# jwwangchn/BONAI

Measured on AMD Instinct MI355X. Metric: training img/s at 1024x1024 LOFT R50-FPN, higher is better.
Workload: dtype bf16; 1 GPU; LOFT R50-FPN + FOA, 8x1024x1024 synthetic tiles per GPU (BASELINE configs[1]), 80 gt/img, full train step (fwd+losses+bwd+allreduce+clip+SGD), random-init weights, RoI heads at the load of a trained RPN (first proposals = jittered gt boxes); global_batch=8, per_gpu_batch=8, parallelism=dp1, graph_features=False

## Files before the change

### bonai_amd/csrc/elementwise.hip

```cpp
#include "loft_common.h"
#include "../../include/loft_hip.h"
#include "conv_tap.h"

__device__ __forceinline__ void ld8(const bf16_t* p, float v[8]) {
    uint4 t = *reinterpret_cast<const uint4*>(p);
    unpack8_16(t, v);
}
__device__ __forceinline__ void st8(bf16_t* p, const float v[8]) {
    *reinterpret_cast<uint4*>(p) = pack8_16(v);
}

__device__ __forceinline__ void ld8(const float* p, float v[8]) { ld4(p, v); ld4(p + 4, v + 4); }
__device__ __forceinline__ void st8(float* p, const float v[8]) { st4(p, v); st4(p + 4, v + 4); }

static inline dim3 ew_grid(long nvec) {
    long b = (nvec + 255) / 256;
    if (b > 8192) b = 8192;
    if (b < 1) b = 1;
    return dim3((unsigned)b);
}

__global__ void relu_bwd_kernel(const bf16_t* __restrict__ g, const bf16_t* __restrict__ y, bf16_t* __restrict__ out,
                                long nvec) {
    for (long i = blockIdx.x * (long)blockDim.x + threadIdx.x; i < nvec; i += (long)gridDim.x * blockDim.x) {
// ... 625 lines not shown
        const int mid = (lo + hi) >> 1;
        if (e0 < t.end[mid]) hi = mid; else lo = mid + 1;
    }
    while (lo < t.S - 1 && e >= t.end[lo]) ++lo;
    return lo;
}

template <bool NEST, bool TAIL>
__device__ __forceinline__ void sgd_elem(float& pv, float& mv, const float gv, const float s, const float lr, const float mu,
                                         const float wd) {
#pragma clang fp contract(off)
    float d, upd;
    if (TAIL) {
        d = __builtin_fmaf(gv, s, wd * pv);
        mv = mu * mv + d;
        upd = NEST ? d + mu * mv : mv;
    } else {
        d = __builtin_fmaf(wd, pv, gv * s);
        mv = __builtin_fmaf(mu, mv, d);
        upd = NEST ? __builtin_fmaf(mu, mv, d) : mv;
    }
    pv = __builtin_fmaf(-lr, upd, pv);
}
template <bool SEG, bool NEST>
__device__ __forceinline__ void sgd_update(float* __restrict__ p, const float* __restrict__ g, float* __restrict__ m, long n,
                                           float gnorm_sq, float max_norm, float lr, float mu, float wd, float gscale,
                                           const SegTable tab, const long stride, const long t0) {
    float clip = 1.f;
    if (max_norm > 0.f) {
        const float norm = sqrtf(gnorm_sq) * gscale;
        if (norm > max_norm) clip = max_norm / (norm + 1e-6f);
    }
    const float s = clip * gscale;
    const bool al = ((reinterpret_cast<uintptr_t>(p) | reinterpret_cast<uintptr_t>(g) | reinterpret_cast<uintptr_t>(m)) & 15) == 0;
    const long n4 = al ? n >> 2 : 0;
    float4* p4 = reinterpret_cast<float4*>(p);
    float4* m4 = reinterpret_cast<float4*>(m);
    const float4* g4 = reinterpret_cast<const float4*>(g);
    const long lane = threadIdx.x & 63;
    auto rates = [&](long e, long first, float& lr_e, float& wd_e) {
        lr_e = lr; wd_e = wd;
        if (SEG) {
            const int sg = seg_find(tab, e, first);
            lr_e = lr * tab.lr_mult[sg]; wd_e = wd * tab.wd_mult[sg];
        }
    };
    auto upd = [&](float4& pv, float4& mv, const float4 gv, long i) {
        float lr_e, wd_e;
        rates(4 * i, 4 * (i - lane), lr_e, wd_e);
        sgd_elem<NEST, false>(pv.x, mv.x, gv.x, s, lr_e, mu, wd_e);
        sgd_elem<NEST, false>(pv.y, mv.y, gv.y, s, lr_e, mu, wd_e);
        sgd_elem<NEST, false>(pv.z, mv.z, gv.z, s, lr_e, mu, wd_e);
        sgd_elem<NEST, false>(pv.w, mv.w, gv.w, s, lr_e, mu, wd_e);
    };
    long i = t0;
    for (; i + stride < n4; i += 2 * stride) {
// ... 265 lines not shown
    if (bias_out && blockIdx.x == 0)
        for (int n = threadIdx.x; n < CoutP; n += blockDim.x) {
            if (n >= Cout) bias_out[n] = 0.f;
            else if (gamma) bias_out[n] = beta[n] - mean[n] * gamma[n] * rsqrtf(var[n] + eps);
            else bias_out[n] = cbias ? cbias[n] : 0.f;
        }
}
LOFT_EXPORT int loft_fold_pack(const float* w, const float* conv_bias, const float* gamma, const float* beta, const float* mean,
                               const float* var, float eps, int Cout, int Cin, int RS, void* wp_fwd, void* wp_dgrad,
                               float* bias_out, int pack_f32, int CoutP, int CinP, void* stream) {
    if (CoutP < Cout || CinP < Cin) return (int)hipErrorInvalidValue;
    const long total = (long)CoutP * CinP * RS;
    if (total <= 0) return 0;
    if (pack_f32)
        hipLaunchKernelGGL(fold_pack_kernel<float>, ew_grid(total), dim3(256), 0, (hipStream_t)stream, w, conv_bias, gamma, beta,
                           mean, var, eps, Cout, Cin, RS, (float*)wp_fwd, (float*)wp_dgrad, bias_out, CoutP, CinP);
    else
        hipLaunchKernelGGL(fold_pack_kernel<bf16_t>, ew_grid(total), dim3(256), 0, (hipStream_t)stream, w, conv_bias, gamma, beta,
                           mean, var, eps, Cout, Cin, RS, (bf16_t*)wp_fwd, (bf16_t*)wp_dgrad, bias_out, CoutP, CinP);
    LOFT_LAUNCH_CHECK();
    return 0;
}

__device__ __forceinline__ int find_record(const long* __restrict__ desc, int n, long key) {
    int cnt = 0;
    for (int j = threadIdx.x & 63; j < n; j += 64) cnt += desc[(long)j * 16 + 15] <= key ? 1 : 0;
    for (int o = 32; o > 0; o >>= 1) cnt += __shfl_xor(cnt, o, 64);
    return cnt - 1;
}

constexpr int FOLD_CHUNK = 2048;
constexpr int FOLD_TILE_MAX_RS = 9;
constexpr int FOLD_NT_TAPS = 32, FOLD_NT_TAPS_LOG2 = 5;
constexpr int FOLD_TILE_FLOATS = FOLD_NT_TAPS * (64 * FOLD_TILE_MAX_RS + 4) / 2;
__global__ __launch_bounds__(256) void fold_pack_multi_kernel(const long* __restrict__ desc, int n, long nchunks) {
    __shared__ float tile[FOLD_TILE_FLOATS];
    for (long c = blockIdx.x; c < nchunks; c += gridDim.x) {
        const int lo = find_record(desc, n, c);
        const long* d = desc + (long)lo * 16;
        const float* w = reinterpret_cast<const float*>(d[0]);
        const float* cbias = reinterpret_cast<const float*>(d[1]);
        const float* gamma = reinterpret_cast<const float*>(d[2]);
        const float* beta = reinterpret_cast<const float*>(d[3]);
        const float* mean = reinterpret_cast<const float*>(d[4]);
        const float* var = reinterpret_cast<const float*>(d[5]);
        bf16_t* wp = reinterpret_cast<bf16_t*>(d[6]);
        bf16_t* wpt = reinterpret_cast<bf16_t*>(d[7]);
        float* bias_out = reinterpret_cast<float*>(d[8]);
        const float eps = __int_as_float((int)d[9]);
        const int Cout = (int)d[10], Cin = (int)d[11], CoutP = (int)d[13], CinP = (int)d[14];
        const bool nmajor = d[12] < 0;
        const int RS = (int)(nmajor ? -d[12] : d[12]);
        const int local_chunk = (int)(c - d[15]);
        if (local_chunk == 0 && bias_out)
            for (int nn = threadIdx.x; nn < CoutP; nn += blockDim.x) {
                if (nn >= Cout) bias_out[nn] = 0.f;
                else if (gamma) bias_out[nn] = beta[nn] - mean[nn] * gamma[nn] * rsqrtf(var[nn] + eps);
                else bias_out[nn] = cbias ? cbias[nn] : 0.f;
            }
        if (nmajor) {
            bf16_t* row = reinterpret_cast<bf16_t*>(tile);
            const int nn = local_chunk, per = Cin * RS;
            const float sc = gamma ? gamma[nn] * rsqrtf(var[nn] + eps) : 1.f;
            __syncthreads();
            const unsigned rs_mul = RS == 1 ? 0u : 0xFFFFFFFFu / (unsigned)RS + 1u;
            const bool small = per < 65536;
            for (int j = threadIdx.x; j < per; j += 256) {
                const int cc = RS == 1 ? j : (small ? (int)__umulhi((unsigned)j, rs_mul) : j / RS), t = j - cc * RS;
                row[t * Cin + cc] = f32_to_bf16(w[(long)nn * per + j] * sc);
            }
            __syncthreads();
            if (wp)
                for (int j = threadIdx.x * 2; j < per; j += 512)
                    *reinterpret_cast<uint32_t*>(wp + (long)nn * per + j) = *reinterpret_cast<const uint32_t*>(row + j);
            continue;
        }
        if (RS > FOLD_TILE_MAX_RS) {
            const long total = (long)CoutP * CinP * RS;
            const long i0 = (long)local_chunk * FOLD_CHUNK;
            for (long i = i0 + threadIdx.x; i < i0 + FOLD_CHUNK && i < total; i += blockDim.x) {
                const int cc = (int)(i % CinP);
                const long r = i / CinP;
                const int nn = (int)(r % CoutP), t = (int)(r / CoutP);
                float v = 0.f;
                if (nn < Cout && cc < Cin) {
                    v = w[((long)nn * Cin + cc) * RS + t];
                    if (gamma) v *= gamma[nn] * rsqrtf(var[nn] + eps);
                }
                const bf16_t h = f32_to_bf16(v);
                if (wp) wp[i] = h;
                if (wpt) wpt[((long)t * CinP + cc) * CoutP + nn] = h;
            }
            continue;
        }
        bf16_t* bt = reinterpret_cast<bf16_t*>(tile);
        const int NT = RS == 1 ? 64 : FOLD_NT_TAPS;
        const int tc = (CinP + 63) >> 6;
        const int n0 = (local_chunk / tc) * NT, c0 = (local_chunk % tc) * 64;
        const int span = 64 * RS, ldw = span + 4;
        __syncthreads();
        const bool vec = (Cin & 63) == 0 && (CinP & 7) == 0 && (CoutP & 7) == 0 && (reinterpret_cast<uintptr_t>(w) & 15) == 0;
        const unsigned rs_mul = RS == 1 ? 0u : 0xFFFFFFFFu / (unsigned)RS + 1u;
        if (vec) {
            const int q4 = span >> 2;
            const unsigned q_mul = 0xFFFFFFFFu / (unsigned)q4 + 1u;
            for (int i = threadIdx.x; i < NT * q4; i += 256) {
                const int row = (int)__umulhi((unsigned)i, q_mul), off = (i - row * q4) << 2;
                const int nn = n0 + row;
                float4 v = make_float4(0.f, 0.f, 0.f, 0.f);
                if (nn < Cout) {
                    v = *reinterpret_cast<const float4*>(w + ((long)nn * Cin + c0) * RS + off);
                    if (gamma) { const float sc = gamma[nn] * rsqrtf(var[nn] + eps); v.x *= sc; v.y *= sc; v.z *= sc; v.w *= sc; }
                }
                uint2 pk;
                pk.x = (uint32_t)f32_to_bf16(v.x) | ((uint32_t)f32_to_bf16(v.y) << 16);
                pk.y = (uint32_t)f32_to_bf16(v.z) | ((uint32_t)f32_to_bf16(v.w) << 16);
                *reinterpret_cast<uint2*>(bt + row * ldw + off) = pk;
            }
        } else {
            const unsigned sp_mul = 0xFFFFFFFFu / (unsigned)span + 1u;
            for (int i = threadIdx.x; i < NT * span; i += 256) {
                const int row = (int)__umulhi((unsigned)i, sp_mul), off = i - row * span;
                const int nn = n0 + row, cc = c0 + (RS == 1 ? off : (int)__umulhi((unsigned)off, rs_mul));
                float v = 0.f;
                if (nn < Cout && cc < Cin) {
                    v = w[((long)nn * Cin + c0) * RS + off];
                    if (gamma) v *= gamma[nn] * rsqrtf(var[nn] + eps);
                }
                bt[row * ldw + off] = f32_to_bf16(v);
            }
        }
        __syncthreads();
        const int ntsh = RS == 1 ? 6 : FOLD_NT_TAPS_LOG2;
        if (wp && vec) {
            for (int i = threadIdx.x; i < RS * NT * 8; i += 256) {
                const int l8 = i & 7, r2 = i >> 3, row = r2 & (NT - 1), t = r2 >> ntsh;
                const int nn = n0 + row;
                if (nn < CoutP) {
                    const bf16_t* tp = bt + row * ldw + (8 * l8) * RS + t;
                    uint32_t q[4];
#pragma unroll
                    for (int k = 0; k < 4; ++k) q[k] = (uint32_t)tp[(2 * k) * RS] | ((uint32_t)tp[(2 * k + 1) * RS] << 16);
                    *reinterpret_cast<uint4*>(wp + ((long)t * CoutP + nn) * CinP + c0 + 8 * l8) = make_uint4(q[0], q[1], q[2], q[3]);
                }
            }
        } else if (wp) {
            for (int i = threadIdx.x; i < RS * NT * 32; i += 256) {
                const int cp = i & 31, r2 = i >> 5, row = r2 & (NT - 1), t = r2 >> ntsh;
                const int nn = n0 + row, cc = c0 + 2 * cp;
                if (nn < CoutP && cc < CinP) {
// ... 8 lines not shown
                const int g8 = i & (gp - 1), r2 = i >> gsh, ccl = r2 & 63, t = r2 >> 6;
                const int nn = n0 + 8 * g8;
                if (nn < CoutP) {
                    const bf16_t* tp = bt + (8 * g8) * ldw + ccl * RS + t;
                    uint32_t q[4];
#pragma unroll
                    for (int k = 0; k < 4; ++k) q[k] = (uint32_t)tp[(2 * k) * ldw] | ((uint32_t)tp[(2 * k + 1) * ldw] << 16);
                    *reinterpret_cast<uint4*>(wpt + ((long)t * CinP + c0 + ccl) * CoutP + nn) = make_uint4(q[0], q[1], q[2], q[3]);
                }
            }
        } else if (wpt) {
            const int hsh = ntsh - 1, hp = 1 << hsh;
            for (int i = threadIdx.x; i < RS * 64 * hp; i += 256) {
                const int np = i & (hp - 1), r2 = i >> hsh, ccl = r2 & 63, t = r2 >> 6;
                const int nn = n0 + 2 * np, cc = c0 + ccl;
                if (nn < CoutP && cc < CinP) {
                    const bf16_t* tp = bt + 2 * np * ldw + ccl * RS + t;
                    *reinterpret_cast<uint32_t*>(wpt + ((long)t * CinP + cc) * CoutP + nn) = (uint32_t)tp[0] | ((uint32_t)tp[ldw] << 16);
                }
            }
        }
    }
}
LOFT_EXPORT int loft_fold_pack_multi(const int64_t* desc, int n, int64_t nchunks, void* stream) {
    if (n <= 0 || nchunks <= 0) return 0;
    long blocks = nchunks < 16384 ? nchunks : 16384;
    hipLaunchKernelGGL(fold_pack_multi_kernel, dim3((unsigned)blocks), dim3(256), 0, (hipStream_t)stream, (const long*)desc, n,
                       (long)nchunks);
    LOFT_LAUNCH_CHECK();
    return 0;
}

__global__ __launch_bounds__(256) void transpose_bf16_kernel(const bf16_t* __restrict__ src, bf16_t* __restrict__ dst, int R, int Cc) {
    __shared__ bf16_t t[64][66];
    const int r0 = blockIdx.y * 64, c0 = blockIdx.x * 64;
    for (int i = threadIdx.x; i < 64 * 32; i += 256) {
        const int r = i >> 5, cp = (i & 31) * 2;
        uint32_t v = 0;
        if (r0 + r < R && c0 + cp < Cc) v = *reinterpret_cast<const uint32_t*>(src + (long)(r0 + r) * Cc + c0 + cp);
        t[r][cp] = (bf16_t)(v & 0xffff);
        t[r][cp + 1] = (bf16_t)(v >> 16);
    }
    __syncthreads();
    for (int i = threadIdx.x; i < 64 * 32; i += 256) {
        const int c = i >> 5, rp = (i & 31) * 2;
        if (c0 + c < Cc && r0 + rp < R)
            *reinterpret_cast<uint32_t*>(dst + (long)(c0 + c) * R + r0 + rp) = (uint32_t)t[rp][c] | ((uint32_t)t[rp + 1][c] << 16);
    }
}
LOFT_EXPORT int loft_transpose_bf16(const void* src, void* dst, int R, int Cc, void* stream) {
    if (R <= 0 || Cc <= 0) return 0;
    if ((R & 1) || (Cc & 1)) return (int)hipErrorInvalidValue;
// ... 442 lines not shown
```

### bonai_amd/debug.py

```python
import contextlib
import os

SWITCHES = {
    'no_side_stream': 'mask / bbox branches, the RPN proposal chain and the backbone weight gradients all on the main stream '
                      '(the mode of bench.py\'s roofline instrumentation)',
    'no_bbox_side_stream': 'the bbox head on the main stream (the mask branch keeps its side stream)',
    'no_rpn_side_stream': 'the RPN proposal chain (sort, decode, NMS) on the main stream',
    'no_rpn_target_prefetch': 'RPN anchor assignment + sampling after the RPN convs on the main stream, not beside the backbone',
    'no_rpn_loss_stream': 'the RPN losses (and with them the sparse RPN backward) on the main stream',
    'no_wgrad_stream': 'backbone weight-gradient launches on the data-gradient stream',
    'unpack_stream': 'the batched weight-gradient unpack launches (descriptor upload + loft_fold_unpack_bwd_multi) on a stream of their '
                     'own instead of on the main stream between the data-gradient kernels (round 6: measured, not the default)',
    'no_prepack': 'BN fold + operand packing per conv per step instead of one launch per step (kernels.PrepackRegistry)',
    'no_unpack_queue': 'one loft_fold_unpack_bwd launch per conv instead of the batched unpack (kernels.UnpackQueue)',
    'no_grad_sink': 'gradients returned to autograd and accumulated by it, not deposited in the arena by the kernels',
    'no_leaf_sink': 'narrow heads and the sparse RPN backward return their parameter gradients to autograd (per-parameter accumulation '
                    'launches) instead of depositing them through the unpack queue (nn._queue_param_grads)',
    'no_head_fusion': 'narrow 1x1 heads (RPN objectness + deltas, mask logits) as launches of their own instead of in the producing '
                      'conv\'s epilogue (loft_conv_tap_bf16_head)',
    'no_grad_join': 'autograd sums the two data gradients of a backbone stage output (next stage + FPN lateral) with an elementwise add '
                    'instead of the residual block taking the lateral\'s deposit as its data-gradient residual (nn.JOIN)',
    'no_deconv_fusion': 'the mask head\'s 2x2 deconvolution as four parity launches instead of one launch whose four channel tiles are '
                        'the four taps (loft_deconv2x2_bf16: the input tile read once)',
    'no_zero_pool': 'torch.zeros / torch.empty per accumulation buffer instead of the step\'s pre-zeroed / scratch slabs',
    'no_feat_hub': 'autograd sums the RPN / RoI-extractor gradients of the FPN maps (no shared per-level gradient map)',
    'no_block_fusion': 'one autograd node per conv of a residual block instead of nn.res_block',
    'no_linear_fn': 'Linear layers through the generic conv node',
    'no_bneck_fusion': 'the frozen / inference 64-plane bottleneck as three (four) tap-conv launches instead of conv1 + the fused tail '
                       '(loft_bneck_tail_bf16: 3x3 + 1x1 expansion + shortcut + ReLU in one launch)',
    'no_pair_fusion': 'the last 1x1 of bottleneck k and the first 1x1 of bottleneck k+1 (layer2 / layer3) as two launches each way instead '
                      'of one (loft_bneck_pair_bf16: the block output is written once and not re-read as the next conv1\'s operand)',
    'wgrad_no_patch': 'the tap weight-gradient kernel for 64-channel high-resolution layers (no patch kernel)',
    'roi_fp32_bwd': 'RoIAlign backward into fp32 maps + a cast',
    'roi_sort': 'RoIAlign forward workgroups in (image, level, row strip) launch order for lists of >= 256 RoIs (loft_roi_order; '
                'measured neutral on the step, not shipped)',
    'no_roi_sort': 'list (sampling) order even where kernels.ROI_FWD_SORT_MIN asks for the launch order',
# ... 28 lines not shown
```

### bonai_amd/engine.py

```python
import os

import torch
import torch.distributed as dist

from . import kernels as K
from .debug import DBG
from .loss_scale import parse_loss_scale


class FlatArena:

    def __init__(self, model):
        self.params = [p for p in model.parameters() if p.requires_grad]
        dev = self.params[0].device
        order = list(reversed(self.params))
        self.offsets, off = {}, 0
        for p in order:
            self.offsets[id(p)] = off
            off += (p.numel() + 7) // 8 * 8
        self.numel = off
        self.data = torch.zeros(off, dtype=torch.float32, device=dev)
        self.grad = torch.zeros(off, dtype=torch.float32, device=dev)
        self.momentum = torch.zeros(off, dtype=torch.float32, device=dev)
        for p in order:
# ... 433 lines not shown
                F2.WGRAD_STREAM = self._wgrad_stream
        try:
            if self.scaler is None:
                (out['loss'] if self.loss_scale == 1.0 else out['loss'] * self.loss_scale).backward()
            else:
                (out['loss'] * self._scale).backward()
            if F2.UNPACK_Q is not None:
                F2.UNPACK_Q.flush()
        finally:
            if F2.UNPACK_Q is not None:
                F2.UNPACK_Q.join()
            F2.UNPACK_Q = None
            F2.WGRAD_STREAM = None
            F2.GRAD_SINK = prev
            F2.HUB = None
            F2.JOIN = None
            K.WEIGHT_PLANES = prev_wpl
            K.zero_pool_end()
        self.reducer.finish()
        self.gnorm_sq.zero_()
        K.sumsq_(self.arena.grad, self.gnorm_sq)
        if not self._plain_sgd:
            self._config_optimizer_step(self.lr if lr is None else lr)
        elif self.scaler is None:
            K.sgd_momentum_(self.arena.data, self.arena.grad, self.arena.momentum, self.gnorm_sq, self.max_norm,
                            self.lr if lr is None else lr, self.mu, self.wd, grad_scale=1.0 / (self.world * self.loss_scale))
        else:
            c = self.scaler
            K.sgd_momentum_scaled_(self.arena.data, self.arena.grad, self.arena.momentum, self.gnorm_sq, self.max_norm,
                                   self.lr if lr is None else lr, self.mu, self.wd, 1.0 / self.world, self.scale_state)
            K.loss_scale_update_(self.scale_state, self.gnorm_sq, 1.0 / self.world, c['growth_factor'], c['backoff_factor'],
                                 c['growth_interval'], c['min_scale'], c['max_scale'])
        self.iter += 1
        self._steps_run += 1
        return out
```

### bonai_amd/kernels.py

```python
import ctypes
import os

import numpy as np
import torch

from . import lib as L
from .debug import DBG as _DBG

c_int, c_int64, c_float, c_void_p = ctypes.c_int, ctypes.c_int64, ctypes.c_float, ctypes.c_void_p


def h2d(values, dtype, device):
    t = torch.from_numpy(values).to(dtype) if isinstance(values, np.ndarray) else torch.tensor(values, dtype=dtype)
    if torch.device(device).type != 'cuda':
        return t.to(device)
    if H2D_KEEP is not None:
        global _H2D_STREAM
        for _ in range(64):
            if _H2D_STREAM is None:
                _H2D_STREAM = torch.cuda.Stream()
            with torch.cuda.stream(_H2D_STREAM):
                if not torch.cuda.is_current_stream_capturing():
                    break
            _H2D_STREAM = None
# ... 1799 lines not shown
    L.dev_check(w, conv_bias)
    dtype = dtype or L.act16()
    w = w.contiguous()
    Cout, Cin, R, S = w.shape
    T = R * S
    dev = w.device
    CoutP, CinP = cout_pad or Cout, cin_pad or Cin
    wp = out_fwd if out_fwd is not None else (torch.empty(T, CoutP, CinP, dtype=dtype, device=dev) if want_fwd else None)
    wpt = out_dgrad if out_dgrad is not None else (torch.empty(T, CinP, CoutP, dtype=dtype, device=dev) if want_dgrad else None)
    bias = out_bias if out_bias is not None else torch.empty(CoutP, dtype=torch.float32, device=dev)
    g = b = m = v = None
    if bn is not None:
        g, b, m, v = [t.contiguous() for t in bn]
    cb = conv_bias.contiguous() if conv_bias is not None else None
    L.check(lib.loft_fold_pack(L.ptr(w), L.ptr(cb), L.ptr(g), L.ptr(b), L.ptr(m), L.ptr(v), eps, Cout, Cin, T,
                               L.ptr(wp), L.ptr(wpt), L.ptr(bias), int(dtype == torch.float32), CoutP, CinP, L.stream()),
            'loft_fold_pack')
    return wp, wpt, bias


FOLD_CHUNK = 2048
FOLD_TILE_MAX_RS = 9
FOLD_NT_TAPS = 32


class PrepackRegistry:

    def __init__(self):
        self.jobs, self.order = {}, []
        self.desc = None
        self.nchunks = 0
        self.step = -1
        self.k8jobs, self.k8desc = {}, None
        self.f32jobs, self.f32order, self.f32desc = {}, [], None
        self.wplanes = {}

    def request(self, ws, conv_biases, bn, eps, cout_p, cin_p, want_dgrad, flat_chw=None):
        key = (tuple(w.data_ptr() for w in ws), tuple(0 if b is None else b.data_ptr() for b in conv_biases),
               0 if bn is None else (bn[0].data_ptr(), bn[2].data_ptr()), cout_p, cin_p, bool(want_dgrad), flat_chw)
        grp = self.jobs.get(key)
        if grp is None:
            G = len(ws)
            dev = ws[0].device
            if flat_chw is not None:
                C, H, W = flat_chw
                Cout, Cin, RS, T, kin = ws[0].shape[0], C, -(H * W), 1, C * H * W
                cout_p, cin_p = Cout, C
            else:
                Cout, Cin = ws[0].shape[0], ws[0].shape[1]
                RS = T = (ws[0].shape[2] * ws[0].shape[3]) if ws[0].dim() == 4 else 1
                kin = cin_p
            grp = dict(wp=torch.empty(G, T, cout_p, kin, dtype=L.act16(), device=dev),
                       wpt=torch.empty(G, T, kin, cout_p, dtype=L.act16(), device=dev) if want_dgrad else None,
                       bias=torch.empty(G, cout_p, dtype=torch.float32, device=dev), step=-2, members=[], flat=flat_chw)
            for g in range(G):
                grp['members'].append(dict(w=ws[g], cb=conv_biases[g], bn=bn, eps=float(eps), dims=(Cout, Cin, RS, cout_p, cin_p),
                                           wp=grp['wp'][g], wpt=None if grp['wpt'] is None else grp['wpt'][g], bias=grp['bias'][g]))
            self.jobs[key] = grp
            self.order.append(key)
            self.desc = None
        if grp['step'] != self.step:
            for j in grp['members']:
                w4 = j['w']
                if grp['flat'] is not None:
                    C, H, W = grp['flat']
                    w4 = w4.detach().view(-1, C, H, W).permute(0, 2, 3, 1).reshape(w4.shape[0], -1)
                if w4.dim() == 2:
                    w4 = w4.detach().view(w4.shape[0], w4.shape[1], 1, 1)
                cop, cip = (j['dims'][3], j['dims'][4]) if grp['flat'] is None else (w4.shape[0], w4.shape[1])
                fold_pack(w4, j['cb'], j['bn'], j['eps'], want_dgrad=j['wpt'] is not None, out_fwd=j['wp'], out_dgrad=j['wpt'],
                          out_bias=j['bias'], cout_pad=cop, cin_pad=cip)
            grp['step'] = self.step
        return grp['wp'], grp['wpt'], grp['bias']

    def request_f32(self, ws, conv_biases, bn, eps, cout_p, cin_p, want_dgrad):
        key = (tuple(w.data_ptr() for w in ws), tuple(0 if b is None else b.data_ptr() for b in conv_biases),
               0 if bn is None else (bn[0].data_ptr(), bn[2].data_ptr()), cout_p, cin_p, bool(want_dgrad))
        grp = self.f32jobs.get(key)
        if grp is None:
            G, dev = len(ws), ws[0].device
# ... 63 lines not shown
    def _run_f32_cached(self, groups):
        plib = L.load_for(torch.float16)
        fdesc, fb, fn, sdesc, sb, sn = self.f32desc
        L.check(plib.loft_fold_f32_multi(L.ptr(fdesc), fn, fb, L.stream()), 'loft_fold_f32_multi')
        if sn:
            L.check(plib.loft_split_planes_f32_multi(L.ptr(sdesc), sn, sb, L.stream()), 'loft_split_planes_f32_multi')

    def k8(self, m):
        job = self.k8jobs.get(m.data_ptr())
        if job is None:
            owned = any(m.data_ptr() == t.data_ptr() for grp in self.jobs.values() for t in (grp['wp'], grp['wpt']) if t is not None)
            if not owned or m.dim() != 2 or m.shape[1] % 8 or not m.is_contiguous():
                return None
            job = dict(src=m, dst=torch.empty(m.shape[1] // 8, m.shape[0], 8, dtype=m.dtype, device=m.device), step=-2)
            self.k8jobs[m.data_ptr()] = job
            self.k8desc = None
        if job['step'] != self.step:
            pack_k8([job['src']], [job['dst']])
            job['step'] = self.step
        return job['dst']

    def run(self, step):
        self.step = step
        if self.order:
            self._run_16(step)
        if self.f32order:
            groups = [self.f32jobs[k] for k in self.f32order]
            self.f32slots[:self.f32nslots].zero_()
            if self.f32desc is None:
                self.f32desc = self._run_f32(groups, None, zero=False)
            else:
                self._run_f32_cached(groups)
            for grp in groups:
                grp['step'] = step
        if self.k8jobs:
            js = list(self.k8jobs.values())
            _, self.k8desc = pack_k8([j['src'] for j in js], [j['dst'] for j in js], self.k8desc)
            for j in js:
                j['step'] = step

    def _run_16(self, step):
        lib = L.load()
        if self.desc is None:
            import struct
            rows, chunk = [], 0
            for j in (m for key in self.order for m in self.jobs[key]['members']):
                Cout, Cin, RS, CoutP, CinP = j['dims']
                bn = j['bn']
                p = lambda t: 0 if t is None else t.data_ptr()
                eps_bits = struct.unpack('<i', struct.pack('<f', j['eps']))[0]
                rows.append([p(j['w']), p(j['cb']), p(bn[0]) if bn else 0, p(bn[1]) if bn else 0, p(bn[2]) if bn else 0,
                             p(bn[3]) if bn else 0, p(j['wp']), p(j['wpt']), p(j['bias']), eps_bits, Cout, Cin, RS, CoutP, CinP, chunk])
                if RS < 0:
                    chunk += Cout
                elif RS > FOLD_TILE_MAX_RS:
                    chunk += (CoutP * CinP * RS + FOLD_CHUNK - 1) // FOLD_CHUNK
                else:
                    nt = 64 if RS == 1 else FOLD_NT_TAPS
                    chunk += ((CoutP + nt - 1) // nt) * ((CinP + 63) // 64)
            self.nchunks = chunk
            dev = self.jobs[self.order[0]]['wp'].device
            self.desc = h2d(rows, torch.int64, dev)
            self.nrows = len(rows)
        L.check(lib.loft_fold_pack_multi(L.ptr(self.desc), self.nrows, self.nchunks, L.stream()), 'loft_fold_pack_multi')
        for key in self.order:
            grp = self.jobs[key]
            if grp['flat'] is not None and grp['wpt'] is not None:
                for j in grp['members']:
                    O, Kd = j['wp'].shape[-2], j['wp'].shape[-1]
                    L.check(lib.loft_transpose_bf16(L.ptr(j['wp']), L.ptr(j['wpt']), O, Kd, L.stream()), 'loft_transpose_bf16')
        for key in self.order:
            self.jobs[key]['step'] = step



_LOSS_SCRATCH = {}


def _loss_view(t, row_dims):
    dims = [(int(n), int(st)) for n, st in zip(t.shape[:row_dims], t.stride()[:row_dims]) if n != 1]
    merged = []
    for n, st in dims:
        if merged and merged[-1][1] == st * n:
            merged[-1] = (merged[-1][0] * n, st)
        else:
            merged.append((n, st))
    if len(merged) > 3:
        return None
    while len(merged) < 3:
        merged.insert(0, (1, 0))
    (_, s0), (d1, s1), (d2, s2) = merged
    if d1 == 1 and d2 == 1:
        return 1, 1, s2 if merged[2][0] != 1 or s2 else 1, 0, 0
    return d1, d2, s0, s1, s2

# ... 309 lines not shown
```

### include/loft_hip.h

```cpp
#ifndef LOFT_HIP_H
#define LOFT_HIP_H
#include <stdint.h>

#ifdef __cplusplus
extern "C" {
#endif

#define LOFT_F32 0
#define LOFT_BF16 1
#define LOFT_F16 2
int loft_act16_dtype(void);

int loft_roi_align_fwd(const void* const* feats_host, const int* H_host, const int* W_host, const float* scales_host,
                       int num_levels, int finest_scale, int C, int dtype, const float* rois, int K, int P,
                       int n_rot, void* out, void* stream);
int loft_roi_align_bwd(void* const* grad_feats_host, const int* H_host, const int* W_host, const float* scales_host,
                       int num_levels, int finest_scale, int C, int dtype, const float* rois, int K, int P,
                       int n_rot, const void* grad_out, int B, int accumulate, int rois_sorted, void* workspace,
                       int grad_dtype, void* stream);
#define LOFT_ROI_AUTO 0
#define LOFT_ROI_FWD_SAMPLE 1
#define LOFT_ROI_FWD_SEP4 2
#define LOFT_ROI_BWD_VALU 1
#define LOFT_ROI_BWD_PIPE 2
// ... 311 lines not shown
                          int backward, void* stream);
int loft_avgpool(const void* src, void* dst, int dtype, int B, int Ho, int Wo, int C, int shift, int backward, int accumulate,
                 void* stream);
int loft_stem3x3s2_bn_relu(const float* img, const float* w, const float* scale, const float* shift, void* out, int dtype,
                           int B, int H, int W, void* stream);
int loft_stem3x3s2_wgrad(const float* img, const void* g, const void* y, float* dwp, float* db, int dtype, int B, int H, int W,
                         void* stream);
int loft_stem7x7_pool_wgrad(const float* img, const void* y, const void* gp, float* dwp, float* db, int dtype, int B, int H,
                            int W, void* stream);

int loft_mdcn_sample_fwd(const void* x, const float* offmask, void* col, int dtype, int B, int IH, int IW, int C, int OH,
                         int OW, int kh, int kw, int stride, int pad, int dil, int deform_groups, int offmask_stride,
                         void* stream);
int loft_mdcn_sample_bwd(const void* x, const float* offmask, const void* dcol, float* dx, float* doffmask, int dtype, int B,
                         int IH, int IW, int C, int OH, int OW, int kh, int kw, int stride, int pad, int dil,
                         int deform_groups, int offmask_stride, void* workspace, void* stream);
int64_t loft_mdcn_bwd_workspace_bytes(int B, int C, int OH, int OW, int kh, int kw, int stride, int dil, int deform_groups,
                                      int offmask_stride);

int loft_fold_pack(const float* w, const float* conv_bias, const float* gamma, const float* beta, const float* mean,
                   const float* var, float eps, int Cout, int Cin, int RS, void* wp_fwd, void* wp_dgrad, float* bias_out,
                   int pack_f32, int CoutP, int CinP, void* stream);
int loft_fold_pack_multi(const int64_t* desc, int n, int64_t nchunks, void* stream);
int loft_fold_f32_multi(const int64_t* desc, int n, int64_t nblocks, void* stream);
int loft_split_planes_f32_multi(const int64_t* desc, int n, int64_t nblocks, void* stream);
int loft_fold_unpack_bwd_multi(const int64_t* desc, int njobs, int64_t nblocks, int lds_floats, void* stream);
int loft_transpose_bf16(const void* src, void* dst, int R, int Cc, void* stream);
int loft_fold_unpack_bwd(const float* dwp, const float* db, const float* w, const float* gamma, const float* mean,
                         const float* var, float eps, int Cout, int Cin, int RS, float* dw, float* dgamma, float* dbeta,
                         int CoutP, int CinP, int accumulate, void* stream);

int loft_narrow_head_bwd(const float* g, int g_stride, const void* x, const float* w, int64_t M, int Cin, int Cout,
                         int relu_in, void* gx, float* dw, float* db, void* stream);
int loft_narrow_head_bwd_f32(const float* g, int g_stride, const float* x, const float* w, int64_t M, int Cin, int Cout,
                             int relu_in, float* gx, float* dw, float* db, void* stream);

int64_t loft_random_sample_workspace_bytes(int B, int N);
int loft_random_sample(const int64_t* gt_inds, int B, int N, int num, int max_pos, int mode, uint64_t seed,
                       int64_t* pos_idx, uint8_t* pos_valid, int64_t* neg_idx, uint8_t* neg_valid, void* workspace, void* stream);

int loft_rpn_sample_gather(const void* const* heads, const int* H, const int* W, const int64_t* lvl_off, int num_levels,
                           int B, int Cp, int A, const float* anchors, const float* gts, int Kmax,
                           const int64_t* gt_inds, int64_t N, const int64_t* pos_idx, const uint8_t* pos_valid, int P,
                           const int64_t* neg_idx, const uint8_t* neg_valid, int Q, const float* means_host,
                           const float* stds_host, float* vals, int32_t* rows, int64_t* slot, float* tgt,
                           int64_t* label, float* weight, void* stream);
// ... 24 lines not shown
```

Baseline: 238.6 img/s.

## Fuse SGD momentum step with next step's BN-fold weight prepack

The optimizer update is merged with the per-step BN fold and bf16 operand packing. Conv weights inside the parameter arena are updated by SGD as they are read for packing, and the remaining parameter ranges are updated by a separate range kernel. This removes one full read/write pass over conv weights and the separate pack launch at the start of the next step. In exchange it adds planning logic, version checks for freshness, and a fallback path for members that cannot be fused.

Result: no change. 239.3 img/s, median of 5 (+0.3%).

```diff
diff --git a/bonai_amd/csrc/elementwise.hip b/bonai_amd/csrc/elementwise.hip
--- a/bonai_amd/csrc/elementwise.hip
+++ b/bonai_amd/csrc/elementwise.hip
@@ -671,16 +671,19 @@
     }
     pv = __builtin_fmaf(-lr, upd, pv);
 }
+__device__ __forceinline__ float sgd_grad_factor(float gnorm_sq, float max_norm, float gscale) {
+    float clip = 1.f;
+    if (max_norm > 0.f) {
+        const float norm = sqrtf(gnorm_sq) * gscale;
+        if (norm > max_norm) clip = max_norm / (norm + 1e-6f);
+    }
+    return clip * gscale;
+}
 template <bool SEG, bool NEST>
 __device__ __forceinline__ void sgd_update(float* __restrict__ p, const float* __restrict__ g, float* __restrict__ m, long n,
                                            float gnorm_sq, float max_norm, float lr, float mu, float wd, float gscale,
                                            const SegTable tab, const long stride, const long t0) {
-    float clip = 1.f;
-    if (max_norm > 0.f) {
-        const float norm = sqrtf(gnorm_sq) * gscale;
-        if (norm > max_norm) clip = max_norm / (norm + 1e-6f);
-    }
-    const float s = clip * gscale;
+    const float s = sgd_grad_factor(gnorm_sq, max_norm, gscale);
     const bool al = ((reinterpret_cast<uintptr_t>(p) | reinterpret_cast<uintptr_t>(g) | reinterpret_cast<uintptr_t>(m)) & 15) == 0;
     const long n4 = al ? n >> 2 : 0;
     float4* p4 = reinterpret_cast<float4*>(p);
@@ -992,9 +995,10 @@
     return 0;
 }
 
+template <int WIDTH = 16, int COL = 15>
 __device__ __forceinline__ int find_record(const long* __restrict__ desc, int n, long key) {
     int cnt = 0;
-    for (int j = threadIdx.x & 63; j < n; j += 64) cnt += desc[(long)j * 16 + 15] <= key ? 1 : 0;
+    for (int j = threadIdx.x & 63; j < n; j += 64) cnt += desc[(long)j * WIDTH + COL] <= key ? 1 : 0;
     for (int o = 32; o > 0; o >>= 1) cnt += __shfl_xor(cnt, o, 64);
     return cnt - 1;
 }
@@ -1003,8 +1007,50 @@
 constexpr int FOLD_TILE_MAX_RS = 9;
 constexpr int FOLD_NT_TAPS = 32, FOLD_NT_TAPS_LOG2 = 5;
 constexpr int FOLD_TILE_FLOATS = FOLD_NT_TAPS * (64 * FOLD_TILE_MAX_RS + 4) / 2;
-__global__ __launch_bounds__(256) void fold_pack_multi_kernel(const long* __restrict__ desc, int n, long nchunks) {
-    __shared__ float tile[FOLD_TILE_FLOATS];
+struct FoldLoadPlain {
+    __device__ __forceinline__ float w1(const float* __restrict__ w, long i) const { return w[i]; }
+    __device__ __forceinline__ float4 w4(const float* __restrict__ w, long i) const { return *reinterpret_cast<const float4*>(w + i); }
+    __device__ __forceinline__ float par(const float* __restrict__ q, int i) const { return q[i]; }
+};
+struct FoldLoadSgd {
+    float* p; const float* g; float* m;
+    long n, body_end;
+    float s, lr, mu, wd;
+    bool skip;
+    __device__ __forceinline__ bool inside(const float* q) const { return q >= p && q < p + n; }
+    __device__ __forceinline__ float step(long e, bool store) const {
+        float pv = p[e];
+        if (skip) return pv;
+        float mv = m[e];
+        if (e < body_end) sgd_elem<false, false>(pv, mv, g[e], s, lr, mu, wd);
+        else sgd_elem<false, true>(pv, mv, g[e], s, lr, mu, wd);
+        if (store) { m[e] = mv; p[e] = pv; }
+        return pv;
+    }
+    __device__ __forceinline__ float w1(const float* w, long i) const { return inside(w) ? step((w - p) + i, true) : w[i]; }
+    __device__ __forceinline__ float par(const float* q, int i) const { return inside(q) ? step((q - p) + i, false) : q[i]; }
+    __device__ __forceinline__ float4 w4(const float* w, long i) const {
+        if (!inside(w)) return *reinterpret_cast<const float4*>(w + i);
+        const long e = (w - p) + i;
+        float4 pv = *reinterpret_cast<const float4*>(p + e);
+        if (skip) return pv;
+        if (e >= body_end) {
+            pv.x = step(e, true); pv.y = step(e + 1, true); pv.z = step(e + 2, true); pv.w = step(e + 3, true);
+            return pv;
+        }
+        float4 mv = *reinterpret_cast<const float4*>(m + e);
+        const float4 gv = *reinterpret_cast<const float4*>(g + e);
+        sgd_elem<false, false>(pv.x, mv.x, gv.x, s, lr, mu, wd);
+        sgd_elem<false, false>(pv.y, mv.y, gv.y, s, lr, mu, wd);
+        sgd_elem<false, false>(pv.z, mv.z, gv.z, s, lr, mu, wd);
+        sgd_elem<false, false>(pv.w, mv.w, gv.w, s, lr, mu, wd);
+        *reinterpret_cast<float4*>(m + e) = mv;
+        *reinterpret_cast<float4*>(p + e) = pv;
+        return pv;
+    }
+};
+template <class LD>
+__device__ __forceinline__ void fold_pack_multi_body(const long* __restrict__ desc, int n, long nchunks, float* tile, const LD ld) {
     for (long c = blockIdx.x; c < nchunks; c += gridDim.x) {
         const int lo = find_record(desc, n, c);
         const long* d = desc + (long)lo * 16;
@@ -1025,19 +1071,19 @@
         if (local_chunk == 0 && bias_out)
             for (int nn = threadIdx.x; nn < CoutP; nn += blockDim.x) {
                 if (nn >= Cout) bias_out[nn] = 0.f;
-                else if (gamma) bias_out[nn] = beta[nn] - mean[nn] * gamma[nn] * rsqrtf(var[nn] + eps);
-                else bias_out[nn] = cbias ? cbias[nn] : 0.f;
+                else if (gamma) bias_out[nn] = ld.par(beta, nn) - mean[nn] * ld.par(gamma, nn) * rsqrtf(var[nn] + eps);
+                else bias_out[nn] = cbias ? ld.par(cbias, nn) : 0.f;
             }
         if (nmajor) {
             bf16_t* row = reinterpret_cast<bf16_t*>(tile);
             const int nn = local_chunk, per = Cin * RS;
-            const float sc = gamma ? gamma[nn] * rsqrtf(var[nn] + eps) : 1.f;
+            const float sc = gamma ? ld.par(gamma, nn) * rsqrtf(var[nn] + eps) : 1.f;
             __syncthreads();
             const unsigned rs_mul = RS == 1 ? 0u : 0xFFFFFFFFu / (unsigned)RS + 1u;
             const bool small = per < 65536;
             for (int j = threadIdx.x; j < per; j += 256) {
                 const int cc = RS == 1 ? j : (small ? (int)__umulhi((unsigned)j, rs_mul) : j / RS), t = j - cc * RS;
-                row[t * Cin + cc] = f32_to_bf16(w[(long)nn * per + j] * sc);
+                row[t * Cin + cc] = f32_to_bf16(ld.w1(w, (long)nn * per + j) * sc);
             }
             __syncthreads();
             if (wp)
@@ -1054,8 +1100,8 @@
                 const int nn = (int)(r % CoutP), t = (int)(r / CoutP);
                 float v = 0.f;
                 if (nn < Cout && cc < Cin) {
-                    v = w[((long)nn * Cin + cc) * RS + t];
-                    if (gamma) v *= gamma[nn] * rsqrtf(var[nn] + eps);
+                    v = ld.w1(w, ((long)nn * Cin + cc) * RS + t);
+                    if (gamma) v *= ld.par(gamma, nn) * rsqrtf(var[nn] + eps);
                 }
                 const bf16_t h = f32_to_bf16(v);
                 if (wp) wp[i] = h;
@@ -1079,8 +1125,8 @@
                 const int nn = n0 + row;
                 float4 v = make_float4(0.f, 0.f, 0.f, 0.f);
                 if (nn < Cout) {
-                    v = *reinterpret_cast<const float4*>(w + ((long)nn * Cin + c0) * RS + off);
-                    if (gamma) { const float sc = gamma[nn] * rsqrtf(var[nn] + eps); v.x *= sc; v.y *= sc; v.z *= sc; v.w *= sc; }
+                    v = ld.w4(w, ((long)nn * Cin + c0) * RS + off);
+                    if (gamma) { const float sc = ld.par(gamma, nn) * rsqrtf(var[nn] + eps); v.x *= sc; v.y *= sc; v.z *= sc; v.w *= sc; }
                 }
                 uint2 pk;
                 pk.x = (uint32_t)f32_to_bf16(v.x) | ((uint32_t)f32_to_bf16(v.y) << 16);
@@ -1094,8 +1140,8 @@
                 const int nn = n0 + row, cc = c0 + (RS == 1 ? off : (int)__umulhi((unsigned)off, rs_mul));
                 float v = 0.f;
                 if (nn < Cout && cc < Cin) {
-                    v = w[((long)nn * Cin + c0) * RS + off];
-                    if (gamma) v *= gamma[nn] * rsqrtf(var[nn] + eps);
+                    v = ld.w1(w, ((long)nn * Cin + c0) * RS + off);
+                    if (gamma) v *= ld.par(gamma, nn) * rsqrtf(var[nn] + eps);
                 }
                 bt[row * ldw + off] = f32_to_bf16(v);
             }
@@ -1150,12 +1196,101 @@
         }
     }
 }
+__global__ __launch_bounds__(256) void fold_pack_multi_kernel(const long* __restrict__ desc, int n, long nchunks) {
+    __shared__ float tile[FOLD_TILE_FLOATS];
+    fold_pack_multi_body(desc, n, nchunks, tile, FoldLoadPlain{});
+}
 LOFT_EXPORT int loft_fold_pack_multi(const int64_t* desc, int n, int64_t nchunks, void* stream) {
     if (n <= 0 || nchunks <= 0) return 0;
     long blocks = nchunks < 16384 ? nchunks : 16384;
     hipLaunchKernelGGL(fold_pack_multi_kernel, dim3((unsigned)blocks), dim3(256), 0, (hipStream_t)stream, (const long*)desc, n,
                        (long)nchunks);
     LOFT_LAUNCH_CHECK();
+    return 0;
+}
+
+__device__ __forceinline__ bool sgd_repack_prologue(const float* __restrict__ gnorm_sq, float max_norm, float gscale,
+                                                    const float* __restrict__ ls_state, float& s) {
+    const float ss = *gnorm_sq;
+    bool skip = false;
+    if (ls_state) {
+        skip = ls_nonfinite(ss);
+        gscale = gscale * (1.0f / ls_state[LOFT_LS_SCALE]);
+    }
+    s = sgd_grad_factor(ss, max_norm, gscale);
+    return skip;
+}
+__global__ __launch_bounds__(256) void sgd_repack_kernel(const long* __restrict__ desc, int nrec, long nchunks, float* p,
+                                                         const float* g, float* m, long n, const float* __restrict__ gnorm_sq,
+                                                         float max_norm, float lr, float mu, float wd, float gscale,
+                                                         const float* __restrict__ ls_state) {
+    __shared__ float tile[FOLD_TILE_FLOATS];
+    FoldLoadSgd ld;
+    ld.p = p; ld.g = g; ld.m = m; ld.n = n; ld.body_end = n & ~3L;
+    ld.lr = lr; ld.mu = mu; ld.wd = wd;
+    ld.skip = sgd_repack_prologue(gnorm_sq, max_norm, gscale, ls_state, ld.s);
+    fold_pack_multi_body(desc, nrec, nchunks, tile, ld);
+}
+constexpr int SGD_RANGE_CHUNK = 4096;
+__global__ __launch_bounds__(256) void sgd_ranges_kernel(const long* __restrict__ rng, int nr, long nchunks, float* __restrict__ p,
+                                                         const float* __restrict__ g, float* __restrict__ m, long n,
+                                                         const float* __restrict__ gnorm_sq, float max_norm, float lr, float mu,
+                                                         float wd, float gscale, const float* __restrict__ ls_state) {
+    float s;
+    if (sgd_repack_prologue(gnorm_sq, max_norm, gscale, ls_state, s)) return;
+    const long body_end = n & ~3L;
+    auto one = [&](long e) {
+        float pv = p[e], mv = m[e];
+        if (e < body_end) sgd_elem<false, false>(pv, mv, g[e], s, lr, mu, wd);
+        else sgd_elem<false, true>(pv, mv, g[e], s, lr, mu, wd);
+        m[e] = mv; p[e] = pv;
+    };
+    for (long c = blockIdx.x; c < nchunks; c += gridDim.x) {
+        const long* r = rng + 3L * find_record<3, 2>(rng, nr, c);
+        const long a = r[0] + (c - r[2]) * SGD_RANGE_CHUNK;
+        long b = a + SGD_RANGE_CHUNK;
+        if (b > r[0] + r[1]) b = r[0] + r[1];
+        if (b > n) b = n;
+        if (a < 0 || a >= b) continue;
+        long a4 = (a + 3) & ~3L, b4 = b & ~3L;
+        if (b4 > body_end) b4 = body_end;
+        if (a4 > b4) a4 = b4 = b;
+        for (long e = a + threadIdx.x; e < a4; e += 256) one(e);
+        for (long e = b4 + threadIdx.x; e < b; e += 256) one(e);
+        for (long v = (a4 >> 2) + threadIdx.x; v < (b4 >> 2); v += 256) {
+            float4 pv = reinterpret_cast<const float4*>(p)[v], mv = reinterpret_cast<const float4*>(m)[v];
+            const float4 gv = reinterpret_cast<const float4*>(g)[v];
+            sgd_elem<false, false>(pv.x, mv.x, gv.x, s, lr, mu, wd);
+            sgd_elem<false, false>(pv.y, mv.y, gv.y, s, lr, mu, wd);
+            sgd_elem<false, false>(pv.z, mv.z, gv.z, s, lr, mu, wd);
+            sgd_elem<false, false>(pv.w, mv.w, gv.w, s, lr, mu, wd);
+            reinterpret_cast<float4*>(m)[v] = mv;
+            reinterpret_cast<float4*>(p)[v] = pv;
+        }
+    }
+}
+LOFT_EXPORT int loft_sgd_repack(const int64_t* desc, int nrec, int64_t nchunks, const int64_t* ranges, int nranges,
+                                int64_t nrange_chunks, float* p, const float* g, float* m, int64_t n, const float* gnorm_sq,
+                                float max_norm, float lr, float momentum, float weight_decay, float grad_scale,
+                                const void* ls_state, void* stream) {
+    if (n <= 0) return 0;
+    if (!gnorm_sq || !p || !g || !m || nrec < 0 || nranges < 0 || (nrec > 0 && !desc) || (nranges > 0 && !ranges) ||
+        ((reinterpret_cast<uintptr_t>(p) | reinterpret_cast<uintptr_t>(g) | reinterpret_cast<uintptr_t>(m)) & 15))
+        return (int)hipErrorInvalidValue;
+    if (nrec > 0 && nchunks > 0) {
+        const long blocks = nchunks < 16384 ? nchunks : 16384;
+        hipLaunchKernelGGL(sgd_repack_kernel, dim3((unsigned)blocks), dim3(256), 0, (hipStream_t)stream, (const long*)desc, nrec,
+                           (long)nchunks, p, g, m, (long)n, gnorm_sq, max_norm, lr, momentum, weight_decay, grad_scale,
+                           (const float*)ls_state);
+        LOFT_LAUNCH_CHECK();
+    }
+    if (nranges > 0 && nrange_chunks > 0) {
+        const long blocks = nrange_chunks < 16384 ? nrange_chunks : 16384;
+        hipLaunchKernelGGL(sgd_ranges_kernel, dim3((unsigned)blocks), dim3(256), 0, (hipStream_t)stream, (const long*)ranges,
+                           nranges, (long)nrange_chunks, p, g, m, (long)n, gnorm_sq, max_norm, lr, momentum, weight_decay,
+                           grad_scale, (const float*)ls_state);
+        LOFT_LAUNCH_CHECK();
+    }
     return 0;
 }
 
diff --git a/bonai_amd/debug.py b/bonai_amd/debug.py
--- a/bonai_amd/debug.py
+++ b/bonai_amd/debug.py
@@ -12,6 +12,8 @@
     'unpack_stream': 'the batched weight-gradient unpack launches (descriptor upload + loft_fold_unpack_bwd_multi) on a stream of their '
                      'own instead of on the main stream between the data-gradient kernels (round 6: measured, not the default)',
     'no_prepack': 'BN fold + operand packing per conv per step instead of one launch per step (kernels.PrepackRegistry)',
+    'no_sgd_repack': 'the optimizer step and the next step\'s operand packs as two kernels (loft_sgd_momentum_f32, then loft_fold_pack_multi at '
+                     'the start of the next step) instead of one pass (loft_sgd_repack)',
     'no_unpack_queue': 'one loft_fold_unpack_bwd launch per conv instead of the batched unpack (kernels.UnpackQueue)',
     'no_grad_sink': 'gradients returned to autograd and accumulated by it, not deposited in the arena by the kernels',
     'no_leaf_sink': 'narrow heads and the sparse RPN backward return their parameter gradients to autograd (per-parameter accumulation '
diff --git a/bonai_amd/engine.py b/bonai_amd/engine.py
--- a/bonai_amd/engine.py
+++ b/bonai_amd/engine.py
@@ -479,15 +479,14 @@
         K.sumsq_(self.arena.grad, self.gnorm_sq)
         if not self._plain_sgd:
             self._config_optimizer_step(self.lr if lr is None else lr)
-        elif self.scaler is None:
-            K.sgd_momentum_(self.arena.data, self.arena.grad, self.arena.momentum, self.gnorm_sq, self.max_norm,
-                            self.lr if lr is None else lr, self.mu, self.wd, grad_scale=1.0 / (self.world * self.loss_scale))
         else:
             c = self.scaler
-            K.sgd_momentum_scaled_(self.arena.data, self.arena.grad, self.arena.momentum, self.gnorm_sq, self.max_norm,
-                                   self.lr if lr is None else lr, self.mu, self.wd, 1.0 / self.world, self.scale_state)
-            K.loss_scale_update_(self.scale_state, self.gnorm_sq, 1.0 / self.world, c['growth_factor'], c['backoff_factor'],
-                                 c['growth_interval'], c['min_scale'], c['max_scale'])
+            self.prepack.sgd_step(self.arena.data, self.arena.grad, self.arena.momentum, self.gnorm_sq, self.max_norm,
+                                  self.lr if lr is None else lr, self.mu, self.wd,
+                                  1.0 / self.world if c is not None else 1.0 / (self.world * self.loss_scale), self.scale_state)
+            if c is not None:
+                K.loss_scale_update_(self.scale_state, self.gnorm_sq, 1.0 / self.world, c['growth_factor'], c['backoff_factor'],
+                                     c['growth_interval'], c['min_scale'], c['max_scale'])
         self.iter += 1
         self._steps_run += 1
         return out
diff --git a/bonai_amd/kernels.py b/bonai_amd/kernels.py
--- a/bonai_amd/kernels.py
+++ b/bonai_amd/kernels.py
@@ -1845,6 +1845,7 @@
 FOLD_CHUNK = 2048
 FOLD_TILE_MAX_RS = 9
 FOLD_NT_TAPS = 32
+SGD_RANGE_CHUNK = 4096
 
 
 class PrepackRegistry:
@@ -1857,6 +1858,9 @@
         self.k8jobs, self.k8desc = {}, None
         self.f32jobs, self.f32order, self.f32desc = {}, [], None
         self.wplanes = {}
+        self.launches = 0
+        self._plan = None
+        self._fresh = None
 
     def request(self, ws, conv_biases, bn, eps, cout_p, cin_p, want_dgrad, flat_chw=None):
         key = (tuple(w.data_ptr() for w in ws), tuple(0 if b is None else b.data_ptr() for b in conv_biases),
@@ -1878,7 +1882,8 @@
                        bias=torch.empty(G, cout_p, dtype=torch.float32, device=dev), step=-2, members=[], flat=flat_chw)
             for g in range(G):
                 grp['members'].append(dict(w=ws[g], cb=conv_biases[g], bn=bn, eps=float(eps), dims=(Cout, Cin, RS, cout_p, cin_p),
-                                           wp=grp['wp'][g], wpt=None if grp['wpt'] is None else grp['wpt'][g], bias=grp['bias'][g]))
+                                           wp=grp['wp'][g], wpt=None if grp['wpt'] is None else grp['wpt'][g], bias=grp['bias'][g],
+                                           flat=flat_chw is not None))
             self.jobs[key] = grp
             self.order.append(key)
             self.desc = None
@@ -1988,8 +1993,9 @@
 
     def run(self, step):
         self.step = step
+        plan = self._take_fresh()
         if self.order:
-            self._run_16(step)
+            self._run_16(step, plan)
         if self.f32order:
             groups = [self.f32jobs[k] for k in self.f32order]
             self.f32slots[:self.f32nslots].zero_()
@@ -2000,43 +2006,155 @@
             for grp in groups:
                 grp['step'] = step
         if self.k8jobs:
-            js = list(self.k8jobs.values())
-            _, self.k8desc = pack_k8([j['src'] for j in js], [j['dst'] for j in js], self.k8desc)
-            for j in js:
+            if plan is None:
+                js = list(self.k8jobs.values())
+                _, self.k8desc = pack_k8([j['src'] for j in js], [j['dst'] for j in js], self.k8desc)
+            else:
+                self._k8_of(plan, 'rest')
+            for j in self.k8jobs.values():
                 j['step'] = step
 
-    def _run_16(self, step):
+    def _members(self):
+        return [m for key in self.order for m in self.jobs[key]['members']]
+
+    @staticmethod
+    def _table(members):
+        import struct
+        rows, chunk = [], 0
+        for j in members:
+            Cout, Cin, RS, CoutP, CinP = j['dims']
+            bn = j['bn']
+            p = lambda t: 0 if t is None else t.data_ptr()
+            eps_bits = struct.unpack('<i', struct.pack('<f', j['eps']))[0]
+            rows.append([p(j['w']), p(j['cb']), p(bn[0]) if bn else 0, p(bn[1]) if bn else 0, p(bn[2]) if bn else 0,
+                         p(bn[3]) if bn else 0, p(j['wp']), p(j['wpt']), p(j['bias']), eps_bits, Cout, Cin, RS, CoutP, CinP, chunk])
+            if RS < 0:
+                chunk += Cout
+            elif RS > FOLD_TILE_MAX_RS:
+                chunk += (CoutP * CinP * RS + FOLD_CHUNK - 1) // FOLD_CHUNK
+            else:
+                nt = 64 if RS == 1 else FOLD_NT_TAPS
+                chunk += ((CoutP + nt - 1) // nt) * ((CinP + 63) // 64)
+        return rows, chunk
+
+    @staticmethod
+    def _transposes(lib, members):
+        for j in members:
+            if j['flat'] and j['wpt'] is not None:
+                O, Kd = j['wp'].shape[-2], j['wp'].shape[-1]
+                L.check(lib.loft_transpose_bf16(L.ptr(j['wp']), L.ptr(j['wpt']), O, Kd, L.stream()), 'loft_transpose_bf16')
+
+    def _run_16(self, step, plan=None):
         lib = L.load()
-        if self.desc is None:
-            import struct
-            rows, chunk = [], 0
-            for j in (m for key in self.order for m in self.jobs[key]['members']):
-                Cout, Cin, RS, CoutP, CinP = j['dims']
-                bn = j['bn']
-                p = lambda t: 0 if t is None else t.data_ptr()
-                eps_bits = struct.unpack('<i', struct.pack('<f', j['eps']))[0]
-                rows.append([p(j['w']), p(j['cb']), p(bn[0]) if bn else 0, p(bn[1]) if bn else 0, p(bn[2]) if bn else 0,
-                             p(bn[3]) if bn else 0, p(j['wp']), p(j['wpt']), p(j['bias']), eps_bits, Cout, Cin, RS, CoutP, CinP, chunk])
-                if RS < 0:
-                    chunk += Cout
-                elif RS > FOLD_TILE_MAX_RS:
-                    chunk += (CoutP * CinP * RS + FOLD_CHUNK - 1) // FOLD_CHUNK
-                else:
-                    nt = 64 if RS == 1 else FOLD_NT_TAPS
-                    chunk += ((CoutP + nt - 1) // nt) * ((CinP + 63) // 64)
-            self.nchunks = chunk
-            dev = self.jobs[self.order[0]]['wp'].device
-            self.desc = h2d(rows, torch.int64, dev)
-            self.nrows = len(rows)
-        L.check(lib.loft_fold_pack_multi(L.ptr(self.desc), self.nrows, self.nchunks, L.stream()), 'loft_fold_pack_multi')
-        for key in self.order:
-            grp = self.jobs[key]
-            if grp['flat'] is not None and grp['wpt'] is not None:
-                for j in grp['members']:
-                    O, Kd = j['wp'].shape[-2], j['wp'].shape[-1]
-                    L.check(lib.loft_transpose_bf16(L.ptr(j['wp']), L.ptr(j['wpt']), O, Kd, L.stream()), 'loft_transpose_bf16')
+        if plan is not None:
+            if plan['rest']:
+                self.launches += 1
+                L.check(lib.loft_fold_pack_multi(L.ptr(plan['rest_desc']), len(plan['rest']), plan['rest_chunks'], L.stream()),
+                        'loft_fold_pack_multi')
+                self._transposes(lib, plan['rest'])
+        else:
+            if self.desc is None:
+                rows, self.nchunks = self._table(self._members())
+                dev = self.jobs[self.order[0]]['wp'].device
+                self.desc = h2d(rows, torch.int64, dev)
+                self.nrows = len(rows)
+            self.launches += 1
+            L.check(lib.loft_fold_pack_multi(L.ptr(self.desc), self.nrows, self.nchunks, L.stream()), 'loft_fold_pack_multi')
+            self._transposes(lib, self._members())
         for key in self.order:
             self.jobs[key]['step'] = step
+
+    def _sgd_plan(self, p):
+        plan = self._plan
+        if plan is not None and plan['key'] == (p.data_ptr(), p.numel(), len(self.order)):
+            return plan
+        base, n = p.data_ptr(), p.numel()
+        inside = lambda t: t is not None and base <= t.data_ptr() < base + 4 * n
+        members = self._members()
+        uses = {}
+        for j in members:
+            if inside(j['w']):
+                uses[j['w'].data_ptr()] = uses.get(j['w'].data_ptr(), 0) + 1
+        fused, rest, owned = [], [], []
+        for j in members:
+            Cout, Cin, RS, CoutP, CinP = j['dims']
+            w = j['w']
+            ok = True
+            if inside(w):
+                ok = (uses[w.data_ptr()] == 1 and w.is_contiguous() and w.dtype == torch.float32
+                      and w.numel() == Cout * Cin * abs(RS) and w.data_ptr() + 4 * w.numel() <= base + 4 * n)
+            if 1 <= RS <= FOLD_TILE_MAX_RS and Cin % 64 == 0 and CinP != Cin:
+                ok = False
+            (fused if ok else rest).append(j)
+            if ok and inside(w):
+                owned.append(((w.data_ptr() - base) // 4, w.numel()))
+        ranges, chunk, at = [], 0, 0
+        for o, cnt in sorted(owned) + [(n, 0)]:
+            if o > at:
+                ranges.append([at, o - at, chunk])
+                chunk += (o - at + SGD_RANGE_CHUNK - 1) // SGD_RANGE_CHUNK
+            at = o + cnt
+        watch, seen = [p], {id(p)}
+        for j in fused:
+            for t in (j['w'], j['cb']) + tuple(j['bn'] or ()):
+                if t is not None and id(t) not in seen:
+                    seen.add(id(t))
+                    watch.append(t)
+        rows, nchunks = self._table(fused)
+        rrows, rchunks = self._table(rest)
+        dev = p.device
+        plan = self._plan = dict(key=(base, n, len(self.order)), fused=fused, rest=rest, watch=watch,
+                                 desc=h2d(rows, torch.int64, dev) if rows else None, nchunks=nchunks,
+                                 rest_desc=h2d(rrows, torch.int64, dev) if rrows else None, rest_chunks=rchunks,
+                                 ranges=h2d(ranges, torch.int64, dev) if ranges else None, nranges=len(ranges), range_chunks=chunk,
+                                 k8=None)
+        return plan
+
+    def _k8_of(self, plan, part):
+        k8 = plan['k8']
+        if k8 is None or k8['n'] != len(self.k8jobs):
+            own = {t.data_ptr() for j in plan['fused'] for t in (j['wp'], j['wpt']) if t is not None}
+            k8 = plan['k8'] = dict(n=len(self.k8jobs), fused=[[j for j in self.k8jobs.values() if j['src'].data_ptr() in own], None],
+                                   rest=[[j for j in self.k8jobs.values() if j['src'].data_ptr() not in own], None])
+        js, desc = k8[part]
+        if js:
+            _, k8[part][1] = pack_k8([j['src'] for j in js], [j['dst'] for j in js], desc)
+
+    def sgd_repack(self, p, g, m, gnorm_sq, max_norm, lr, momentum, weight_decay, grad_scale=1.0, ls_state=None):
+        lib = L.load()
+        L.dev_check(p, g, m, gnorm_sq)
+        if ls_state is not None:
+            L.dev_check(ls_state)
+            _ls_state_check(ls_state)
+        if not (p.is_contiguous() and g.is_contiguous() and m.is_contiguous() and p.dtype == g.dtype == m.dtype == torch.float32
+                and p.numel() == g.numel() == m.numel()):
+            raise L.LoftHipError('sgd_repack: p, g, m are contiguous float32 tensors of one size')
+        plan = self._sgd_plan(p)
+        L.check(lib.loft_sgd_repack(L.ptr(plan['desc']), len(plan['fused']), plan['nchunks'], L.ptr(plan['ranges']), plan['nranges'],
+                                    plan['range_chunks'], L.ptr(p), L.ptr(g), L.ptr(m), p.numel(), L.ptr(gnorm_sq), max_norm, lr, momentum,
+                                    weight_decay, grad_scale, L.ptr(ls_state), L.stream()), 'loft_sgd_repack')
+        self._transposes(lib, plan['fused'])
+        if self.k8jobs:
+            self._k8_of(plan, 'fused')
+        self._fresh = (plan, L.act16(), F32_CONTRACT, [t._version for t in plan['watch']])
+
+    def sgd_step(self, p, g, m, gnorm_sq, max_norm, lr, momentum, weight_decay, grad_scale=1.0, ls_state=None):
+        if self.order and not _DBG.no_sgd_repack and not _DBG.no_prepack:
+            self.sgd_repack(p, g, m, gnorm_sq, max_norm, lr, momentum, weight_decay, grad_scale, ls_state)
+            return
+        self._fresh = None
+        if ls_state is None:
+            sgd_momentum_(p, g, m, gnorm_sq, max_norm, lr, momentum, weight_decay, grad_scale=grad_scale)
+        else:
+            sgd_momentum_scaled_(p, g, m, gnorm_sq, max_norm, lr, momentum, weight_decay, grad_scale, ls_state)
+
+    def _take_fresh(self):
+        f, self._fresh = self._fresh, None
+        if f is None or f[0] is not self._plan or f[0]['key'][2] != len(self.order) or f[1] != L.act16() or f[2] != F32_CONTRACT:
+            return None
+        if f[3] != [t._version for t in f[0]['watch']]:
+            return None
+        return f[0]
 
 
 
diff --git a/include/loft_hip.h b/include/loft_hip.h
--- a/include/loft_hip.h
+++ b/include/loft_hip.h
@@ -357,6 +357,9 @@
                    const float* var, float eps, int Cout, int Cin, int RS, void* wp_fwd, void* wp_dgrad, float* bias_out,
                    int pack_f32, int CoutP, int CinP, void* stream);
 int loft_fold_pack_multi(const int64_t* desc, int n, int64_t nchunks, void* stream);
+int loft_sgd_repack(const int64_t* desc, int nrec, int64_t nchunks, const int64_t* ranges, int nranges, int64_t nrange_chunks,
+                    float* p, const float* g, float* m, int64_t n, const float* gnorm_sq, float max_norm, float lr,
+                    float momentum, float weight_decay, float grad_scale, const void* ls_state, void* stream);
 int loft_fold_f32_multi(const int64_t* desc, int n, int64_t nblocks, void* stream);
 int loft_split_planes_f32_multi(const int64_t* desc, int n, int64_t nblocks, void* stream);
 int loft_fold_unpack_bwd_multi(const int64_t* desc, int njobs, int64_t nblocks, int lds_floats, void* stream);
```
